# gogoex/BulletProofsPlus

Measured on AMD Instinct MI355X. Metric: aggregated range-proof verifies/sec (n=64,m=16), higher is better.
Workload: dtype u32 (30-bit limbs of a 381-bit prime field, v_mad_u64_u32)

## Files before the change

### bulletproofsplus_amd/csrc/ec.hpp

```cpp
#pragma once
#include "field.hpp"

namespace bpp {

struct Bls12381 {
    using Fp = BlsFp;
    using Fr = BlsFr;
    using K = Bls12381Consts;
    static constexpr int ID = 0;
};
struct Secp256k1 {
    using Fp = SecpFp;
    using Fr = SecpFr;
    using K = Secp256k1Consts;
    static constexpr int ID = 1;
};

template <class C>
constexpr int jac_words() {
    return 3 * C::Fp::N;
}

template <class C>
struct Aff {
    Fe<typename C::Fp> x, y;
    BPP_HD bool is_inf() const { return x.is_zero() && y.is_zero(); }
};

template <class C>
struct Jac {
    Fe<typename C::Fp> X, Y, Z;
    BPP_HD bool is_inf() const { return Z.is_zero(); }
};

template <class C>
BPP_HD Aff<C> aff_inf() {
    Aff<C> r;
    r.x = Fe<typename C::Fp>::zero();
    r.y = Fe<typename C::Fp>::zero();
    return r;
}
template <class C>
BPP_HD Jac<C> jac_inf() {
    Jac<C> r;
    r.X = Fe<typename C::Fp>::one();
    r.Y = Fe<typename C::Fp>::one();
    r.Z = Fe<typename C::Fp>::zero();
    return r;
}
template <class C>
BPP_HD Jac<C> jac_from_aff(const Aff<C>& p) {
    if (p.is_inf()) return jac_inf<C>();
    Jac<C> r;
// ... 237 lines not shown
    F Pp = fe_sub_nr<6>(U2, p.X);
    F R = fe_csub_nr<4>(S2, neg, p.Y);
    const F PP = fe_sqr_io(Pp);
    const F PPP = fe_mul(Pp, PP);
    const F Q = fe_mul(p.X, PP);
    const F u = fe_add_dbl_nr(PPP, Q);
    const F X3 = fe_sub_nr<4>(fe_sqr_io(R), u);
    const F T = fe_sub_nr<6>(Q, X3);
    const F nY = fe_sub_nr<2>(F::zero(), p.Y);
    const F ZZ3 = fe_mul(p.ZZ, PP);
#if defined(BPP_LAZY_CHECK) && !defined(__HIP_DEVICE_COMPILE__)
    BPP_LAZY_CHECK(fe_below_kp<2>(U2) && fe_below_kp<2>(S2) && fe_below_kp<8>(Pp) && fe_below_kp<6>(R) &&
                   fe_below_kp<2>(PP) && fe_below_kp<2>(PPP) && fe_below_kp<2>(Q) && fe_below_kp<4>(u) &&
                   fe_below_kp<6>(X3) && fe_below_kp<8>(T) && fe_below_kp<3>(nY) && fe_below_kp<2>(ZZ3));
#endif
    if (ZZ3.is_zero()) {
        if (fe_is_zero_mod<5>(R)) {
            Aff<C> qq;
            qq.x = qx;
            qq.y = neg ? fe_sub_nr<1>(F::zero(), qy) : qy;
            p = xyzz_dbl_aff(qq);
        } else {
            p = xyzz_inf<C>();
        }
        return;
    }
    p.Y = fe_mul_add(R, T, nY, PPP);
    p.X = X3;
    p.ZZZ = fe_mul(p.ZZZ, PPP);
    p.ZZ = ZZ3;
}

template <class C>
BPP_HD Jac<C> xyzz_to_jac(const Xyzz<C>& p) {
    if (p.is_inf()) return jac_inf<C>();
    Jac<C> r;
    r.X = fe_mul(p.X, p.ZZ);
    r.Y = fe_mul(p.Y, p.ZZZ);
    r.Z = p.ZZ;
    return r;
}

template <class C>
BPP_HD bool jac_is_identity_class(const Jac<C>& p) {
    return p.is_inf();
}

template <class C>
BPP_HD bool aff_in_prime_subgroup(const Aff<C>& p) {
    if constexpr (C::ID == 0) {
        using F = Fe<typename C::Fp>;
        if (p.is_inf()) return true;
        Jac<C> t = jac_inf<C>();
        for (int i = 63; i >= 0; i--) {
            t = jac_dbl(t);
            if ((C::K::ZABS >> i) & 1ull) t = jac_madd(t, p);
        }
        {
            const Jac<C> base = t;
            Jac<C> acc = jac_inf<C>();
            for (int i = 63; i >= 0; i--) {
                acc = jac_dbl(acc);
                if ((C::K::ZABS >> i) & 1ull) acc = jac_add(acc, base);
            }
            t = acc;
        }
// ... 244 lines not shown
    using F = Fe<typename C::Fp>;
    if (p.is_inf() || q.is_inf()) return p.is_inf() && q.is_inf();
    F Z1Z1 = fe_sqr(p.Z), Z2Z2 = fe_sqr(q.Z);
    if (fe_mul(p.X, Z2Z2) != fe_mul(q.X, Z1Z1)) return false;
    return fe_mul(fe_mul(p.Y, q.Z), Z2Z2) == fe_mul(fe_mul(q.Y, p.Z), Z1Z1);
}

template <class C>
BPP_HD Aff<C> aff_load(const uint32_t* w) {
    Aff<C> r;
    r.x = fe_load<typename C::Fp>(w);
    r.y = fe_load<typename C::Fp>(w + C::Fp::N);
    return r;
}
template <class C>
BPP_HD void aff_store(const Aff<C>& p, uint32_t* w) {
    fe_store(p.x, w);
    fe_store(p.y, w + C::Fp::N);
}
template <class C>
BPP_HD Jac<C> jac_load(const uint32_t* w) {
    Jac<C> r;
    r.X = fe_load<typename C::Fp>(w);
    r.Y = fe_load<typename C::Fp>(w + C::Fp::N);
    r.Z = fe_load<typename C::Fp>(w + 2 * C::Fp::N);
    return r;
}
template <class C>
BPP_HD void jac_store(const Jac<C>& p, uint32_t* w) {
    fe_store(p.X, w);
    fe_store(p.Y, w + C::Fp::N);
    fe_store(p.Z, w + 2 * C::Fp::N);
}

template <class C>
BPP_HD bool aff_from_wire(const uint32_t* w, Aff<C>& out) {
    constexpr int N = C::Fp::N;
    if (w[2 * N] | w[2 * N + 1]) {
        out = aff_inf<C>();
        return true;
    }
    if (!words_lt_mod<typename C::Fp>(w) || !words_lt_mod<typename C::Fp>(w + N)) return false;
    out.x = fe_from_canonical<typename C::Fp>(w);
    out.y = fe_from_canonical<typename C::Fp>(w + N);
    if (out.is_inf()) return false;
    return aff_on_curve(out);
}
template <class C>
BPP_HD void aff_to_wire(const Aff<C>& p, uint32_t* w) {
    constexpr int N = C::Fp::N;
    if (p.is_inf()) {
#pragma unroll
        for (int i = 0; i < 2 * N + 2; i++) w[i] = 0;
        w[2 * N] = 1;
        return;
    }
    fe_to_canonical(p.x, w);
    fe_to_canonical(p.y, w + N);
    w[2 * N] = 0;
    w[2 * N + 1] = 0;
}

template <class C>
BPP_HD Jac<C> aff_mul_words(const Aff<C>& p, const uint32_t* k, int nwords) {
    Jac<C> acc = jac_inf<C>();
    int top = nwords * 32 - 1;
// ... 10 lines not shown
```

### bulletproofsplus_amd/csrc/ed25519.hpp

```cpp
#pragma once
#include "ec.hpp"

namespace bpp {

struct Ed25519 {
    using Fp = EdFp;
    using Fr = EdFr;
    using K = Ed25519Consts;
    static constexpr int ID = 2;
};

template <>
constexpr int jac_words<Ed25519>() {
    return 4 * EdFp::N;
}

template <>
struct Aff<Ed25519> {
    Fe<EdFp> x, y;
    BPP_HD bool is_inf() const { return x.is_zero() && y == Fe<EdFp>::one(); }
};
template <>
struct Jac<Ed25519> {
    Fe<EdFp> X, Y, Z, T;
// ... 136 lines not shown
BPP_HD Xyzz<Ed25519> xyzz_dbl_aff(const Aff<Ed25519>& q) {
    Xyzz<Ed25519> r;
    r.e = aff_dbl(q);
    return r;
}
BPP_HD Xyzz<Ed25519> xyzz_madd(const Xyzz<Ed25519>& p, const Aff<Ed25519>& q) {
    Xyzz<Ed25519> r;
    r.e = jac_madd(p.e, q);
    return r;
}
BPP_HD void xyzz_madd_lazy(Xyzz<Ed25519>& p, const Aff<Ed25519>& q, bool neg) {
    using F = ed::F;
    Jac<Ed25519>& e = p.e;
    const F qm = fe_sub_nr<1>(q.y, q.x);
    const F qp = fe_add_nr(q.y, q.x);
    const F a1 = fe_sub_nr<2>(e.Y, e.X);
    const F b1 = fe_add_nr(e.Y, e.X);
    const F A = fe_mul(a1, ed::select(neg, qp, qm));
    const F B = fe_mul(b1, ed::select(neg, qm, qp));
    const F C = fe_mul(fe_mul(e.T, ed::konst(Ed25519Consts::D2)), fe_mul(q.x, q.y));
    const F D = fe_add_nr(e.Z, e.Z);
    F E = fe_sub_nr<2>(B, A);
    const F H = fe_add_nr(B, A);
    const F Fm = fe_sub_nr<2>(D, C);
    const F Gp = fe_add_nr(D, C);
    F Fq = ed::select(neg, Gp, Fm);
    F G = ed::select(neg, Fm, Gp);
    e.X = fe_mul_io(E, Fq);
    e.T = fe_mul(E, H);
    e.Y = fe_mul_io(G, H);
    e.Z = fe_mul(Fq, G);
}
BPP_HD Jac<Ed25519> xyzz_to_jac(const Xyzz<Ed25519>& p) { return p.e; }

template <>
BPP_HD Jac<Ed25519> jac_load<Ed25519>(const uint32_t* w) {
    constexpr int N = EdFp::N;
    Jac<Ed25519> r;
    r.X = fe_load<EdFp>(w);
    r.Y = fe_load<EdFp>(w + N);
    r.Z = fe_load<EdFp>(w + 2 * N);
    r.T = fe_load<EdFp>(w + 3 * N);
    return r;
}
BPP_HD void jac_store(const Jac<Ed25519>& p, uint32_t* w) {
    constexpr int N = EdFp::N;
    fe_store(p.X, w);
    fe_store(p.Y, w + N);
    fe_store(p.Z, w + 2 * N);
    fe_store(p.T, w + 3 * N);
}

template <>
BPP_HD bool aff_from_wire<Ed25519>(const uint32_t* w, Aff<Ed25519>& out) {
    constexpr int N = EdFp::N;
    if (w[2 * N] | w[2 * N + 1]) {
        out = aff_inf<Ed25519>();
        return true;
    }
    if (!words_lt_mod<EdFp>(w) || !words_lt_mod<EdFp>(w + N)) return false;
    out.x = fe_from_canonical<EdFp>(w);
    out.y = fe_from_canonical<EdFp>(w + N);
    return aff_on_curve(out);
}

}
```

### bulletproofsplus_amd/csrc/impl_msm.hpp

```cpp
#pragma once
#include "hash_to_group.hpp"
#include "host_util.hpp"
#include "pippenger.hpp"

namespace bpp {

template <class P>
__global__ void __launch_bounds__(64) k_dbg_field(int op, const uint32_t* a, const uint32_t* b, uint32_t* out, size_t n) {
    const size_t i = (size_t)blockIdx.x * blockDim.x + threadIdx.x;
    if (i >= n) return;
    uint32_t wa[P::N], wb[P::N], wr[P::N];
    for (int t = 0; t < P::N; t++) {
        wa[t] = a[i * P::N + t];
        wb[t] = b[i * P::N + t];
    }
    Fe<P> x = fe_from_canonical<P>(wa), y = fe_from_canonical<P>(wb), r;
    switch (op) {
        case 0: r = fe_mul(x, y); break;
        case 1: r = fe_add(x, y); break;
        case 2: r = fe_sub(x, y); break;
        case 3: r = fe_inv(x); break;
        case 4: r = fe_sqr(x); break;
        default: r = fe_neg(x); break;
    }
    fe_to_canonical(r, wr);
    for (int t = 0; t < P::N; t++) out[i * P::N + t] = wr[t];
}

template <class C>
__global__ void __launch_bounds__(64) k_dbg_point(int op, const uint32_t* a, const uint32_t* b, uint32_t* out, size_t n) {
    constexpr int WW = 2 * C::Fp::N + 2;
    const size_t i = (size_t)blockIdx.x * blockDim.x + threadIdx.x;
    if (i >= n) return;
    uint32_t wa[WW], wb[WW], wr[WW];
    for (int t = 0; t < WW; t++) {
        wa[t] = a[i * WW + t];
        wb[t] = b[i * WW + t];
    }
    Aff<C> p, q;
    aff_from_wire<C>(wa, p);
    aff_from_wire<C>(wb, q);
    Jac<C> r;
    switch (op) {
        case 0: r = jac_add(jac_from_aff(p), jac_from_aff(q)); break;
        case 1: r = jac_madd(jac_from_aff(p), q); break;
        case 2: r = jac_dbl(jac_from_aff(p)); break;
        case 3: r = jac_madd(jac_dbl(jac_from_aff(p)), q); break;
        case 4: r = jac_add(jac_dbl(jac_from_aff(p)), jac_dbl(jac_from_aff(q))); break;
        default: {
            Xyzz<C> acc = xyzz_inf<C>();
            acc = xyzz_madd(acc, p);
            acc = xyzz_madd(acc, q);
            acc = xyzz_madd(acc, p);
            r = xyzz_to_jac(acc);
            break;
        }
    }
    aff_to_wire(jac_to_aff(r), wr);
    for (int t = 0; t < WW; t++) out[i * WW + t] = wr[t];
}

template <class C>
struct MsmImpl {
    static constexpr int N = C::Fp::N;
    static constexpr int JW = jac_words<C>();
    static constexpr int WW = 2 * N + 2;
    static constexpr int PW = WW / 2;

    static int msm_batch_dev(const uint32_t* d_scalars, const uint32_t* d_points, const std::vector<uint64_t>& offsets,
                             uint64_t* out, hipStream_t st);

    static constexpr size_t PIPPENGER_MIN_N = 4096;
    static size_t msm_workspace_bytes(size_t n, int window_bits);
    static int msm_device(const uint32_t* d_scalars, const uint32_t* d_wire_points, size_t n, int window_bits,
                          uint32_t* d_out_wire, uint32_t* d_status, void* d_ws, size_t ws_bytes, hipStream_t st,
                          bpp_ctx* ctx = nullptr);

    static int msm_pippenger(const uint64_t* scalars, const uint64_t* points, size_t n, int window_bits, uint64_t* out);

    static int msm_batch(const uint64_t* scalars, const uint64_t* points, const uint32_t* lens, size_t count,
                         uint64_t* out);
// ... 317 lines not shown
```

### bulletproofsplus_amd/csrc/impl_prove_batch.hpp

```cpp
#pragma once
#include "impl_verify.hpp"
#include "prover_batch.hpp"

namespace bpp {

template <class C>
struct ProveBatchImpl {
    using V = VerifyImpl<C>;
    static constexpr int JW = V::JW, WW = V::WW;

    struct ProveLayout {
        size_t a, b, cG, cH, pwy, con, vps, part, part1, part2, vout, trst, ch, blind, vals, gams, total;
        size_t chunk;
        unsigned per;
    };
    static size_t prove_chunk(const VerifyShape& s, size_t count) {
        const uint32_t nvp = pb_num_vps(s.k, s.m);
        const size_t chunk_max = std::max<size_t>(1, std::min<size_t>(2048, ((size_t)12 << 30) / ((size_t)nvp * s.N * 32)));
        return std::min(chunk_max, std::max<size_t>(count, 1));
    }
    static ProveLayout prove_layout(const VerifyShape& s, size_t count, bool mixed = false) {
        ProveLayout w;
        const uint32_t nvp = pb_num_vps(s.k, s.m);
        w.chunk = prove_chunk(s, count);
        const size_t nv_total = w.chunk * nvp;
        w.per = blocks_per_proof(s, nv_total);
        const size_t vec = w.chunk * (size_t)s.mn * 32;
        WsCarver o;
        w.a = o.take(vec);
        w.b = o.take(vec);
        w.cG = o.take(vec);
        w.cH = o.take(vec);
        w.pwy = o.take(vec);
        w.con = o.take(w.chunk * (size_t)pb_consts_elems(s.k) * 32);
        w.vps = o.take(nv_total * (size_t)s.N * 32);
        w.part = o.take(nv_total * w.per * FIXED_BLOCK * JW * 4);
        w.part1 = o.take(nv_total * w.per * (FIXED_BLOCK / FOLD_GROUP) * JW * 4);
        w.part2 = o.take(nv_total * w.per * (FIXED_BLOCK / FOLD_GROUP / FOLD_GROUP2) * JW * 4);
        w.vout = o.take(w.chunk * (size_t)s.m * WW * 4);
        w.trst = o.take(w.chunk * 32);
        w.ch = o.take(w.chunk * (size_t)(3 + s.k) * 32);
        w.blind = o.take(w.chunk * (size_t)pb_blind_elems(s.k) * 32);
        w.vals = w.gams = 0;
        if (mixed) {
            w.vals = o.take(w.chunk * (size_t)s.m * 8);
            w.gams = o.take(w.chunk * (size_t)s.m * 32);
        }
        w.total = o.total;
        return w;
    }

    static ProverConsts literals() { return ProverConsts{0, 4, 5, 33, 44, 88, 123, 0}; }
    struct Chunk {
        const VerifyShape& s;
        const ProverConsts& pc;
        const ProveLayout& L;
        uint8_t* ws;
        size_t cnt;
        const uint32_t *blind, *px;
        uint32_t *o_pts, *o_V, *o_sc, *ch;
        hipStream_t st;
        const uint32_t* table;
        uint32_t* w(size_t off) const { return reinterpret_cast<uint32_t*>(ws + off); }
    };
    static void mulvec(const Chunk& c, VpSel sel);
    static const uint32_t* chunk_blinding(const uint32_t* slice, const uint8_t* blind_key, uint64_t index, uint32_t k, size_t cnt,
                                          const uint32_t* px, uint32_t* w_blind, hipStream_t st);
    static void argument(const Chunk& c, bool fs, VpSel literal_sel);

    static int prove_batch_device(bpp_verifier* v, const PassShape& ps, const uint64_t* d_values, const uint64_t* d_gammas,
// ... 59 lines not shown
                                           size_t count, int flags, const uint8_t* blind_key, uint64_t index_base,
                                           uint8_t* out_proofs, uint8_t* out_commitments);
    template <class F>
    static int prove_mixed_staged(const MixedPlan& p, const uint64_t* values, const uint64_t* gammas, size_t wsb, void* out0,
                                  size_t bytes0, void* out1, size_t bytes1, F&& run) {
        size_t nval = 0;
        for (uint32_t c = 0; c < MIXED_CLASSES; c++) nval += p.count[c] << c;
        DevBuf dv, dg, d0, d1, dws;
        HIPCHK(dv.alloc(nval * 8));
        HIPCHK(hipMemcpy(dv.p, values, nval * 8, hipMemcpyHostToDevice));
        int rc = upload_scalars<C>(gammas, nval, dg, nullptr);
        if (rc) return rc;
        HIPCHK(d0.alloc(bytes0));
        HIPCHK(d1.alloc(bytes1));
        HIPCHK(dws.alloc(wsb));
        rc = run(static_cast<const uint64_t*>(dv.p), static_cast<const uint64_t*>(dg.p), d0.p, d1.p, dws.p);
        if (rc) return rc;
        HIPCHK(hipDeviceSynchronize());
        HIPCHK(hipMemcpy(out0, d0.p, bytes0, hipMemcpyDeviceToHost));
        HIPCHK(hipMemcpy(out1, d1.p, bytes1, hipMemcpyDeviceToHost));
        return BPP_OK;
    }
};

#ifdef BPP_IMPL_DEFINITIONS
template <class C>
void ProveBatchImpl<C>::mulvec(const Chunk& c, VpSel sel) {
    const ProveLayout& L = c.L;
    const size_t nv = c.cnt * sel.cnt;
    const unsigned per = std::min(L.per, blocks_per_proof(c.s, nv));
    launch_fixed_msm<C, 2>((unsigned)(nv * per), c.st, c.s, c.w(L.vps), c.table, c.w(L.part), per, 0u, (const uint32_t*)nullptr,
                           (uint32_t*)nullptr, (size_t)0, 0u, sel);
    const size_t f1 = nv * per * (FIXED_BLOCK / FOLD_GROUP), f2 = f1 / FOLD_GROUP2;
    hipLaunchKernelGGL(k_partials_fold<C>, dim3(cdiv(f1, 64)), dim3(64), 0, c.st, c.w(L.part), FOLD_GROUP, c.w(L.part1), f1);
    hipLaunchKernelGGL(k_partials_fold<C>, dim3(cdiv(f2, 64)), dim3(64), 0, c.st, c.w(L.part1), FOLD_GROUP2, c.w(L.part2), f2);
    hipLaunchKernelGGL(k_pb_collect<C>, dim3(cdiv(nv, 64)), dim3(64), 0, c.st, c.s, sel, c.w(L.part2),
                       per * (FIXED_BLOCK / FOLD_GROUP / FOLD_GROUP2), c.o_pts, c.o_V, nv, c.px);
}

template <class C>
const uint32_t* ProveBatchImpl<C>::chunk_blinding(const uint32_t* slice, const uint8_t* blind_key, uint64_t index, uint32_t k,
                                                  size_t cnt, const uint32_t* px, uint32_t* w_blind, hipStream_t st) {
    if (slice || !blind_key) return slice;
    BlindKey bk;
    load_key_words(blind_key, bk.w);
    hipLaunchKernelGGL(k_pb_blind<C>, dim3(cdiv(cnt * pb_blind_elems(k), 64)), dim3(64), 0, st, bk, index, k, w_blind, cnt, px);
    return w_blind;
}

template <class C>
void ProveBatchImpl<C>::argument(const Chunk& c, bool fs, VpSel literal_sel) {
    const VerifyShape& s = c.s;
    const ProveLayout& L = c.L;
    const uint32_t k = s.k, nvp = pb_num_vps(k, s.m);
    const dim3 proofs((unsigned)c.cnt), lanes(cdiv(c.cnt, 64));
    auto round = [&](uint32_t t, uint32_t phase) {
        hipLaunchKernelGGL(k_pb_round<C>, proofs, dim3(256), 0, c.st, s, c.pc, c.blind, t, phase, c.w(L.a), c.w(L.b), c.w(L.cG),
                           c.w(L.cH), c.w(L.pwy), c.w(L.con), c.w(L.vps));
    };
    auto last = [&](uint32_t phase) {
        hipLaunchKernelGGL(k_pb_final<C>, proofs, dim3(256), 0, c.st, s, c.pc, c.blind, phase, c.w(L.a), c.w(L.b), c.w(L.cG),
                           c.w(L.cH), c.w(L.con), c.w(L.vps), c.o_sc, c.px);
    };
    if (!fs) {
        for (uint32_t t = 0; t < k; t++) round(t, PB_ALL);
        last(PB_ALL);
        mulvec(c, literal_sel);
        return;
// ... 213 lines not shown
```

### bulletproofsplus_amd/csrc/impl_verify.hpp

```cpp
#pragma once
#include <functional>
#include <memory>
#include <mutex>

#include "codec.hpp"
#include "combined.hpp"
#include "fixed_launch.hpp"
#include "host_util.hpp"
#include "mixed.hpp"
#include "pippenger.hpp"

enum { BPP_STAGE_FROM_WIRE = 0, BPP_STAGE_SCALARS, BPP_STAGE_FIXED_MSM, BPP_STAGE_VAR_MSM, BPP_STAGE_FINALIZE,
       BPP_NUM_STAGES };
constexpr int BPP_PROFILE_SLOTS = 64;

namespace bpp {
struct PassShape {
    VerifyShape s;
    const uint32_t* challenges;
    TranscriptState tr0;
};
}

struct bpp_verifier {
// ... 22 lines not shown
    }
};

namespace bpp {

inline unsigned blocks_per_proof(const VerifyShape& s, size_t count) {
    const unsigned maxb = cdiv(s.NF, FIXED_BLOCK);
    size_t tpp = ((size_t)1 << 18) / (count ? count : 1);
    tpp = std::max<size_t>(FIXED_BLOCK, std::min<size_t>(tpp, s.NF));
    const unsigned b_lat = cdiv(tpp, FIXED_BLOCK);
    const unsigned b_thr = std::min<unsigned>(cdiv((size_t)32768, count ? count : 1),
                                              std::max<unsigned>(1, s.NF / (FIXED_BLOCK * 4)));
#ifdef BPP_FORCE_PER
    if (count >= 1024) return std::max(1u, std::min<unsigned>(BPP_FORCE_PER, maxb));
#endif
    return std::max(1u, std::min(std::max(b_lat, b_thr), maxb));
}

#ifndef BPP_HORNER_TREE_MAX
#define BPP_HORNER_TREE_MAX 256
#endif
constexpr size_t HORNER_TREE_MAX = BPP_HORNER_TREE_MAX;
constexpr unsigned FOLD_GROUP = 8;
constexpr unsigned FOLD_GROUP2 = 4;

struct WsLayout {
    size_t pts, bad, scalars, prep, fthread, fpart, fpart2, fpart3, vpart, vdig, vwsum, vtbl, vscr, total;
};

template <class C>
struct VerifyImpl {
    static constexpr int N = C::Fp::N;
    static constexpr int JW = jac_words<C>();
    static constexpr int WW = 2 * N + 2;
    static constexpr int PW = WW / 2;

    static WsLayout ws_layout(const VerifyShape& s, size_t count) {
        WsLayout w;
        WsCarver o;
        w.pts = o.take(count * s.NV * 2 * N * 4);
        w.bad = o.take(count * 4);
        w.scalars = o.take(count * (size_t)s.N * 32);
        w.prep = o.take(count * vs_prep_bytes<C>(s));
        w.fthread = o.take(count * blocks_per_proof(s, count) * FIXED_BLOCK * JW * 4);
        w.fpart = o.take(count * blocks_per_proof(s, count) * (FIXED_BLOCK / FOLD_GROUP) * JW * 4);
        w.fpart2 = o.take(count * blocks_per_proof(s, count) * (FIXED_BLOCK / FOLD_GROUP / FOLD_GROUP2) * JW * 4);
        w.fpart3 = o.take(count * (FIXED_BLOCK / FOLD_GROUP / FOLD_GROUP2) * JW * 4);
        w.vpart = o.take(count * JW * 4);
        w.vdig = o.take(count * s.NV * VAR_DIGIT_STRIDE);
        w.vwsum = o.take(count * var_wsums_max<C>() * JW * 4);
        w.vtbl = o.take(count * s.NV * VAR_MULTIPLES * 2 * N * 4);
        w.vscr = o.take(count * s.NV * 2 * (VAR_MULTIPLES - 1) * N * 4);
        w.total = o.total;
        return w;
    }

    static int create(const bpp_ctx& ctx, const uint64_t* gh, const uint64_t* G, const uint64_t* H, size_t n, size_t m,
                      int window_bits, bpp_verifier** out);

    static PassShape own(const bpp_verifier* v) { return PassShape{v->s, v->challenges.u32(), v->tr0}; }
    static PassShape class_shape(const bpp_verifier* v, uint32_t c) {
        return c < v->views.size() ? v->views[c] : own(v);
    }

    static int run(bpp_verifier* v, const PassShape& ps, const uint64_t* d_points, const uint64_t* d_scalars, size_t count,
                   const uint64_t* d_challenges, uint32_t* d_ok, void* d_workspace, size_t workspace_bytes,
                   uint64_t* d_out_scalars, uint64_t* d_out_result, hipStream_t st);
    static int run(bpp_verifier* v, const uint64_t* d_points, const uint64_t* d_scalars, size_t count,
                   const uint64_t* d_challenges, uint32_t* d_ok, void* d_workspace, size_t workspace_bytes,
                   uint64_t* d_out_scalars, uint64_t* d_out_result, hipStream_t st) {
        return run(v, own(v), d_points, d_scalars, count, d_challenges, d_ok, d_workspace, workspace_bytes, d_out_scalars,
                   d_out_result, st);
    }

    static int range_scalars(const PassShape& ps, const uint64_t* d_scalars, const uint64_t* d_challenges, uint32_t* w_sc,
                             size_t count, uint32_t* w_prep, hipStream_t st) {
        const uint32_t* ch = d_challenges ? reinterpret_cast<const uint32_t*>(d_challenges) : ps.challenges;
        const uint32_t ch_stride = d_challenges ? (3 + ps.s.k) * 8 : 0;
        return launch_verify_scalars<C>(ps.s, reinterpret_cast<const uint32_t*>(d_scalars), ch, ch_stride, w_sc, count, w_prep, st);
// ... 559 lines not shown
    v->last_horner_form = lone ? 3u : tree;
    const size_t vlanes = count * (tree == 1 ? var_wsums<C>() * vgroups : var_windows<C>());
    HIPCHK(mark(ev, 2 * BPP_STAGE_VAR_MSM, st));
    hipLaunchKernelGGL(k_var_digits<C>, dim3(cdiv(npts, 256)), dim3(256), 0, st, s, w_sc, w_vd, npts, 0u);
    rc = join_tables(v, st, aux_lock);
    if (rc) return rc;
    hipLaunchKernelGGL(k_var_windows<C>, dim3(cdiv(vlanes, VAR_BLOCK)), dim3(VAR_BLOCK), 0, st, s, w_vd, w_vt, w_vw,
                       vlanes, tree == 1 ? 1u : 0u, vgroups);
    HIPCHK(mark(ev, 2 * BPP_STAGE_VAR_MSM + 1, st));
    return finish(v, s, ws, L, count, w_sc, w_vw, w_bad, d_ok, reinterpret_cast<uint32_t*>(d_out_result), tree, lone, st,
                  ev);
}

template <class C>
int VerifyImpl<C>::finish(bpp_verifier* v, const VerifyShape& s, uint8_t* ws, const WsLayout& L, size_t count,
                          const uint32_t* w_sc, const uint32_t* w_vw, const uint32_t* w_bad, uint32_t* d_ok,
                          uint32_t* d_out_result, uint32_t tree, bool lone, hipStream_t st, hipEvent_t* ev) {
    const unsigned bpp_ = blocks_per_proof(s, count);
    uint32_t* w_fp = reinterpret_cast<uint32_t*>(ws + L.fpart);
    uint32_t* w_vp = reinterpret_cast<uint32_t*>(ws + L.vpart);
    HIPCHK(mark(ev, 2 * BPP_STAGE_FIXED_MSM, st));
    const unsigned hb = tree == 1 ? (unsigned)count : cdiv(count, tree == 2 ? FIXED_BLOCK / 8 : FIXED_BLOCK);
    uint32_t* w_ft = reinterpret_cast<uint32_t*>(ws + L.fthread);
    launch_fixed_msm<C, 0>((unsigned)(hb + count * bpp_), st, s, w_sc, v->table.u32(), w_ft, bpp_, hb, w_vw, w_vp, count,
                           lone ? 3u : tree, VpSel{1u, 0u, 1u, 0u});
    HIPCHK(mark(ev, 2 * BPP_STAGE_FIXED_MSM + 1, st));
    HIPCHK(mark(ev, 2 * BPP_STAGE_FINALIZE, st));
    const unsigned folded = bpp_ * (FIXED_BLOCK / FOLD_GROUP);
    const unsigned folded2 = folded / FOLD_GROUP2;
    uint32_t* w_fp2 = reinterpret_cast<uint32_t*>(ws + L.fpart2);
    if (tree == 1) {
        if (!lone)
            hipLaunchKernelGGL(k_partials_fold<C>, dim3(cdiv(count * folded, 64)), dim3(64), 0, st, w_ft, FOLD_GROUP, w_fp,
                               count * folded);
        hipLaunchKernelGGL(k_finalize_tree<C>, dim3((unsigned)count), dim3(64), 0, st, lone ? w_ft : w_fp,
                           lone ? bpp_ : folded, w_vp, w_bad, d_ok, d_out_result, count);
        HIPCHK(mark(ev, 2 * BPP_STAGE_FINALIZE + 1, st));
        HIPCHK(hipGetLastError());
        return BPP_OK;
    }
    hipLaunchKernelGGL(k_partials_fold<C>, dim3(cdiv(count * folded, 64)), dim3(64), 0, st, w_ft, FOLD_GROUP, w_fp,
                       count * folded);
    hipLaunchKernelGGL(k_partials_fold<C>, dim3(cdiv(count * folded2, 64)), dim3(64), 0, st, w_fp, FOLD_GROUP2, w_fp2,
                       count * folded2);
    const uint32_t* w_last = w_fp2;
    unsigned last = folded2;
    if (bpp_ > 1) {
        uint32_t* w_fp3 = reinterpret_cast<uint32_t*>(ws + L.fpart3);
        last = folded2 / bpp_;
        hipLaunchKernelGGL(k_partials_fold<C>, dim3(cdiv(count * last, 64)), dim3(64), 0, st, w_fp2, bpp_, w_fp3,
                           count * last);
        w_last = w_fp3;
    }
    hipLaunchKernelGGL(k_finalize<C>, dim3(cdiv(count, 64)), dim3(64), 0, st, w_last, last, w_vp, 1u, w_bad, d_ok,
                       d_out_result, count);
    HIPCHK(mark(ev, 2 * BPP_STAGE_FINALIZE + 1, st));
    HIPCHK(hipGetLastError());
    return BPP_OK;
}

template <class C>
int VerifyImpl<C>::run_serialized(bpp_verifier* v, const uint8_t* d_proofs, const uint8_t* d_commitments, size_t count,
                                  bool transcript, uint32_t* d_ok, void* d_workspace, size_t workspace_bytes,
                                  hipStream_t st, uint32_t version, const GroupedArgs* grouped) {
    const VerifyShape& s = v->s;
    if (int rc = container_args_ok(v, version)) return rc;
    const SerLayout L = ser_layout(s, count, grouped ? grouped->group : 0u);
    if (workspace_bytes < L.total) return fail(BPP_E_ARG, "workspace too small");
    uint8_t* ws = static_cast<uint8_t*>(d_workspace);
    uint32_t* w_rec = reinterpret_cast<uint32_t*>(ws + L.records);
    uint32_t* w_sc = reinterpret_cast<uint32_t*>(ws + L.scalars);
    uint32_t* w_st = reinterpret_cast<uint32_t*>(ws + L.status);
    uint64_t* w_ch = reinterpret_cast<uint64_t*>(ws + L.challenges);
    HIPCHK(zero_words_async(w_st, count * 4, st));
    hipLaunchKernelGGL(k_container_decode<C>, dim3(cdiv(count * s.NV, 64)), dim3(64), 0, st, s, d_proofs, d_commitments,
                       w_rec, w_sc, w_st, count, version);
    if constexpr (C::ID == 0)
        hipLaunchKernelGGL(k_records_subgroup<C>, dim3(cdiv(count * s.NV, 64)), dim3(64), 0, st, w_rec, w_st, s.NV,
                           count * s.NV);
    HIPCHK(hipGetLastError());
    if (transcript) {
        int rc = derive_challenges(v, reinterpret_cast<const uint64_t*>(w_rec), count, w_ch, st);
        if (rc) return rc;
    }
// ... 413 lines not shown
```

### bulletproofsplus_amd/csrc/kernels.hpp

```cpp
#pragma once
#include <hip/hip_runtime.h>
#include "ec.hpp"
#include "fixed_glv.hpp"
#include "ed25519.hpp"
#include "ristretto.hpp"
#include "transcript.hpp"

namespace bpp {

constexpr unsigned MSM_BLOCK = 64;
constexpr unsigned VS_PB = 8;
constexpr unsigned VS_BLOCK = VS_PB * 64;
constexpr unsigned FIXED_BLOCK = 128;
constexpr unsigned VAR_BLOCK = 64;
template <class C>
constexpr bool var_glv() {
    return curve_has_glv<C>();
}
template <class C>
constexpr uint32_t var_windows() {
    return var_glv<C>() ? 33u : 65u;
}
template <class C>
constexpr uint32_t var_wsums() {
// ... 50 lines not shown
}

template <class C>
__device__ __forceinline__ Aff<C> aff_ldg(const uint32_t* __restrict__ p) {
    constexpr int N = C::Fp::N;
    constexpr int JW = jac_words<C>();
    uint32_t w[2 * N];
    ld_words<2 * N>(p, w);
    return aff_load<C>(w);
}
template <class C>
__device__ __forceinline__ void aff_stg(uint32_t* __restrict__ p, const Aff<C>& a) {
    constexpr int N = C::Fp::N;
    constexpr int JW = jac_words<C>();
    uint32_t w[2 * N];
    aff_store(a, w);
    st_words<2 * N>(p, w);
}
template <class C>
__device__ __forceinline__ Jac<C> jac_ldg(const uint32_t* __restrict__ p) {
    constexpr int N = C::Fp::N;
    constexpr int JW = jac_words<C>();
    uint32_t w[JW];
    ld_words<JW>(p, w);
    return jac_load<C>(w);
}
template <class C>
__device__ __forceinline__ void jac_stg(uint32_t* __restrict__ p, const Jac<C>& a) {
    constexpr int N = C::Fp::N;
    constexpr int JW = jac_words<C>();
    uint32_t w[JW];
    jac_store(a, w);
    st_words<JW>(p, w);
}

template <class C>
__device__ __forceinline__ Jac<C> block_reduce_jac(Jac<C> acc, uint32_t* lds) {
    constexpr int N = C::Fp::N;
    constexpr int JW = jac_words<C>();
    const int tid = threadIdx.x;
    for (int half = blockDim.x >> 1; half >= 1; half >>= 1) {
        if (tid >= half && tid < 2 * half) jac_store(acc, lds + (size_t)tid * JW);
        __syncthreads();
        if (tid < half) acc = jac_add(acc, jac_load<C>(lds + (size_t)(tid + half) * JW));
        __syncthreads();
    }
    return acc;
}

template <class T>
__device__ __forceinline__ T wave_shfl(const T& v, int src_lane) {
    static_assert(sizeof(T) % 4 == 0, "whole words");
    struct Words {
        uint32_t w[sizeof(T) / 4];
    };
    Words a = __builtin_bit_cast(Words, v);
#pragma unroll
    for (int i = 0; i < (int)(sizeof(T) / 4); i++) a.w[i] = (uint32_t)__shfl((int)a.w[i], src_lane, 64);
    return __builtin_bit_cast(T, a);
}

template <class C>
__device__ __forceinline__ Jac<C> wave_sum_jac(Jac<C> x, int span = 64) {
    const int lane = threadIdx.x & 63;
#pragma unroll 1
    for (int d = span >> 1; d >= 1; d >>= 1) {
// ... 722 lines not shown
__device__ __forceinline__ void glds16(const uint32_t* gsrc, uint32_t lds_byte_addr) {
    unsigned keep;
    lds_byte_addr = __builtin_amdgcn_readfirstlane(lds_byte_addr);
    asm volatile("s_mov_b32 %0, m0\n\ts_mov_b32 m0, %2\n\ts_nop 0\n\tglobal_load_lds_dwordx4 %1, off\n\ts_mov_b32 m0, %0"
                 : "=&s"(keep)
                 : "v"(gsrc), "s"(lds_byte_addr)
                 : "memory");
}

#ifndef BPP_FIXED_RING
#define BPP_FIXED_RING 2
#endif
constexpr int FIXED_RING = BPP_FIXED_RING;
template <class C>
constexpr unsigned fixed_lds_bytes() {
    return (FIXED_BLOCK / 64) * (FIXED_RING * (2 * C::Fp::N / 4) + 2) * 1024;
}

struct VpSel {
    uint32_t nvp, first, cnt, prover;
};

template <class C>
constexpr int fixed_waves() {
    return C::Fp::NL > 9 ? BPP_FIXED_WAVES : 3;
}
template <class C, int ROLE = 0>
__global__ void __launch_bounds__(FIXED_BLOCK, fixed_waves<C>()) k_fixed_msm(VerifyShape s, const uint32_t* __restrict__ scalars,
                            const uint32_t* __restrict__ table, uint32_t* __restrict__ partials, uint32_t per,
                            uint32_t horner_blocks, const uint32_t* __restrict__ wsum, uint32_t* __restrict__ var_out,
                            size_t horner_count, uint32_t horner_tree, VpSel sel) {
    constexpr int N = C::Fp::N;
    constexpr int JW = jac_words<C>();
    constexpr int CH = 2 * N / 4;
    constexpr int WAVE_WORDS = (FIXED_RING * CH + 2) * 256;
    constexpr bool GLV = fixed_glv<C>();
    constexpr int NWD = GLV ? GLV_HALF_WORDS : WIN_FULL_WORDS;
    extern __shared__ __align__(16) uint32_t lds[];
    if (blockIdx.x < horner_blocks) {
        if (horner_tree == 2) {
            const size_t b = (size_t)blockIdx.x * (blockDim.x / 8) + threadIdx.x / 8;
            var_horner_group<C>(wsum, var_out, b, b < horner_count, lds + (size_t)(threadIdx.x >> 6) * 64 * JW);
        } else if (horner_tree) {
            const size_t b = blockIdx.x;
            if constexpr (var_glv<C>()) {
                if (b < horner_count) var_horner_wave2<C>(wsum, var_out, b, lds, horner_tree == 3 ? VAR_GROUPS : 1u);
            } else {
                if (b < horner_count && threadIdx.x < 64) var_horner_wave_ed(wsum, var_out, b, horner_tree == 3 ? VAR_GROUPS : 1u);
            }
        } else {
            const size_t lane = (size_t)blockIdx.x * blockDim.x + threadIdx.x;
            if (lane < horner_count) var_horner_lane<C>(wsum, var_out, lane);
        }
        return;
    }
#ifdef BPP_XCD_REMAP
    uint32_t bid = blockIdx.x - horner_blocks;
    {
        const uint32_t nb = gridDim.x - horner_blocks;
        if (nb % 8 == 0 && horner_blocks % 8 == 0) bid = (bid % 8) * (nb / 8) + bid / 8;
    }
#else
    const uint32_t bid = blockIdx.x - horner_blocks;
#endif
    const size_t b = bid / per;
    const uint32_t part = bid % per;
// ... 148 lines not shown
        dma_scalar(0);
        asm volatile("s_waitcnt vmcnt(0)" ::: "memory");
        take_scalar();
        if (NQ > 1) dma_scalar(G > 1 ? 1u : 0u);
    }
    for (int d = 0; d < FIXED_RING; d++) issue();
    for (uint32_t ph = 0; ph < PH; ph++)
    for (uint32_t t = 0; t < (ph + 1 < PH ? T : TT); t++) {
        if constexpr (GLV) {
            if (ph == 1 && t == 0) xyzz_mul_x_beta(acc);
        }
        const uint32_t slot = (GLV ? ph * T + t : t) % FIXED_RING;
        asm volatile("s_waitcnt vmcnt(%0)" ::"n"((FIXED_RING - 1) * CH) : "memory");
        uint32_t raw[2 * N];
        const uint4* q = reinterpret_cast<const uint4*>(ring + slot * CH * 256);
#pragma unroll
        for (int k = 0; k < CH; k++) {
            const uint4 v = q[k * 64 + lane];
            raw[4 * k] = v.x;
            raw[4 * k + 1] = v.y;
            raw[4 * k + 2] = v.z;
            raw[4 * k + 3] = v.w;
        }
        const bool valid = (vbits >> slot) & 1u, neg = (nbits >> slot) & 1u;
        Aff<C> cur = aff_load<C>(raw);
        if constexpr (GLV) {
            if (ph == 1 && t >= T && ((bbits >> slot) & 1u)) aff_mul_x_beta(cur);
        }
        issue();
        if (valid) xyzz_madd_lazy(acc, cur, neg);
    }
    asm volatile("s_waitcnt vmcnt(0)" ::: "memory");
    if (ROLE != 1 && horner_tree != 3) {
        jac_stg<C>(partials + ((size_t)bid * blockDim.x + threadIdx.x) * JW, xyzz_to_jac(acc));
    } else {
        __syncthreads();
        Jac<C> sum = block_reduce_jac<C>(xyzz_to_jac(acc), lds);
        if (threadIdx.x == 0) jac_stg<C>(partials + (size_t)bid * JW, sum);
    }
}

template <class C>
__global__ void __launch_bounds__(64) k_partials_fold(const uint32_t* __restrict__ in, uint32_t group,
                                                      uint32_t* __restrict__ out, size_t n_out) {
    constexpr int JW = jac_words<C>();
    const size_t i = (size_t)blockIdx.x * blockDim.x + threadIdx.x;
    if (i >= n_out) return;
    const uint32_t* src = in + i * group * JW;
    Jac<C> acc = jac_ldg<C>(src);
    for (uint32_t t = 1; t < group; t++) acc = jac_add(acc, jac_ldg<C>(src + (size_t)t * JW));
    jac_stg<C>(out + i * JW, acc);
}


template <class C>
__global__ void __launch_bounds__(256) k_var_digits(VerifyShape s, const uint32_t* __restrict__ scalars,
                                                    uint8_t* __restrict__ digits, size_t items, uint32_t flat) {
    const size_t item = (size_t)blockIdx.x * blockDim.x + threadIdx.x;
    if (item >= items) return;
    const size_t b = item / s.NV;
    const uint32_t v = (uint32_t)(item % s.NV);
    uint32_t k[8];
    ld_words<8>(scalars + (flat ? item : b * s.N + var_term_index(s, v)) * 8, k);
    uint32_t out[VAR_DIGIT_STRIDE / 4];
#pragma unroll
    for (int t = 0; t < (int)(VAR_DIGIT_STRIDE / 4); t++) out[t] = 0;
    if constexpr (var_glv<C>()) {
        uint32_t rem[4], q[4];
        bool nh[2];
        glv_split_signed<C>(k, rem, q, nh[0], nh[1]);
#pragma unroll
        for (int h = 0; h < 2; h++) {
            uint32_t w[5];
            uint32_t carry = 0;
#pragma unroll
            for (int t = 0; t < 5; t++) {
                const uint64_t x = (uint64_t)(t < 4 ? (h ? q[t] : rem[t]) : 0u) + (t < 4 ? 0x88888888u : 0x8u) + carry;
                w[t] = (uint32_t)x;
                carry = (uint32_t)(x >> 32);
            }
#pragma unroll
            for (int j = 0; j < 33; j++) {
                uint32_t nib = (w[j >> 3] >> ((j & 7) * 4)) & 15u;
                if (nh[h]) nib = 16u - nib;
// ... 37 lines not shown
    uint32_t* T = tables + lane * M * 2 * N;
    uint32_t* S = scratch + lane * 2 * (M - 1) * N;
    const Aff<C> p = aff_ldg<C>(proof_pts + lane * 2 * N);
    aff_stg<C>(T, p);
    if (p.is_inf()) {
        for (int k = 1; k < M; k++) aff_stg<C>(T + (size_t)k * 2 * N, p);
        return;
    }
    affine_chain<C>(aff_dbl(p), T, M - 1, T + 2 * N, S);
}

template <class C>
__global__ void __launch_bounds__(VAR_BLOCK, BPP_VAR_WAVES) k_var_windows(VerifyShape s, const uint8_t* __restrict__ digits,
                                                                         const uint32_t* __restrict__ tables,
                                                                         uint32_t* __restrict__ wsum, size_t lanes,
                                                                         uint32_t split, uint32_t groups) {
    constexpr int N = C::Fp::N;
    constexpr int JW = jac_words<C>();
    const size_t lane = (size_t)blockIdx.x * blockDim.x + threadIdx.x;
    if (lane >= lanes) return;
    constexpr uint32_t NW = var_windows<C>();
    constexpr uint32_t H = var_glv<C>() ? 2u : 1u;
    const uint32_t HL = split ? 1u : H;
    const uint32_t per_proof = NW * (H / HL) * groups;
    const size_t b = lane / per_proof;
    const uint32_t g = (uint32_t)(lane % per_proof) / (NW * (H / HL));
    const uint32_t h0 = split ? (uint32_t)(lane / NW) % H : 0u;
    const uint32_t j = (uint32_t)(lane % NW);
    const uint32_t gs = (s.NV + groups - 1) / groups;
    const uint32_t v0 = g * gs, v1 = min(s.NV, v0 + gs);
    const uint8_t* dg = digits + b * s.NV * VAR_DIGIT_STRIDE + j;
    const uint32_t* T = tables + b * s.NV * VAR_MULTIPLES * 2 * N;
    Xyzz<C> acc = xyzz_inf<C>();
    Fe<typename C::Fp> beta;
    if constexpr (var_glv<C>()) {
#pragma unroll
        for (int i = 0; i < C::Fp::NL; i++) beta.l[i] = C::K::BETA[i];
    }
    const uint32_t items = (v1 > v0 ? v1 - v0 : 0u) * HL;
    auto digit_of = [&](uint32_t u) -> int32_t {
        return (int32_t)dg[(size_t)(v0 + u / HL) * VAR_DIGIT_STRIDE + (h0 + u % HL) * NW] - 8;
    };
    auto entry_of = [&](uint32_t u, int32_t d) -> const uint32_t* {
        return T + ((size_t)(v0 + u / HL) * VAR_MULTIPLES + (d < 0 ? -d : d) - 1) * 2 * N;
    };
    uint32_t raw[2 * N];
    int32_t d_next = items ? digit_of(0) : 0;
    if (d_next) ld_words<2 * N>(entry_of(0, d_next), raw);
    for (uint32_t u = 0; u < items; u++) {
        const int32_t d = d_next;
        Aff<C> cur;
        if (d) cur = aff_load<C>(raw);
        if (u + 1 < items) {
            d_next = digit_of(u + 1);
            if (d_next) ld_words<2 * N>(entry_of(u + 1, d_next), raw);
        }
        bool neg = d < 0;
        if constexpr (var_glv<C>()) {
            if (d && ((h0 + u % HL) & 1u)) {
                cur.x = fe_mul(cur.x, beta);
                fe_cond_sub_p(cur.x);
                if (glv_image_negates_y<C>()) neg = !neg;
            }
        }
        if (d) xyzz_madd_lazy(acc, cur, neg);
    }
    jac_stg<C>(wsum + lane * JW, xyzz_to_jac(acc));
}

template <class C>
__global__ void __launch_bounds__(64) k_finalize(const uint32_t* __restrict__ fixed_partials, uint32_t per,
                                                 const uint32_t* __restrict__ var_partials, uint32_t nv,
                                                 const uint32_t* __restrict__ bad, uint32_t* __restrict__ ok,
                                                 uint32_t* __restrict__ wire_result, size_t count) {
    constexpr int N = C::Fp::N;
    constexpr int JW = jac_words<C>();
    const size_t b = (size_t)blockIdx.x * blockDim.x + threadIdx.x;
    if (b >= count) return;
    Jac<C> acc = jac_inf<C>();
    for (uint32_t t = 0; t < per; t++) acc = jac_add(acc, jac_ldg<C>(fixed_partials + (b * per + t) * JW));
    for (uint32_t t = 0; t < nv; t++) acc = jac_add(acc, jac_ldg<C>(var_partials + (b * nv + t) * JW));
    ok[b] = (jac_is_identity_class(acc) && !bad[b]) ? 0u : 1u;
    if (wire_result) {
        uint32_t w[2 * N + 2];
        aff_to_wire(jac_to_aff(acc), w);
#pragma unroll
        for (int t = 0; t < 2 * N + 2; t++) wire_result[b * (2 * N + 2) + t] = w[t];
    }
}

template <class C>
__global__ void __launch_bounds__(64) k_finalize_tree(const uint32_t* __restrict__ fixed_partials, uint32_t per,
                                                      const uint32_t* __restrict__ var_partials,
                                                      const uint32_t* __restrict__ bad, uint32_t* __restrict__ ok,
                                                      uint32_t* __restrict__ wire_result, size_t count) {
    constexpr int N = C::Fp::N;
    constexpr int JW = jac_words<C>();
    __shared__ __align__(16) uint32_t lds[64 * JW];
// ... 18 lines not shown
```

Baseline: 202,500.

## Keep fixed-MSM partials in XYZZ form and batch GLV beta multiply

Fixed-base MSM threads now store their partial sums in XYZZ coordinates and the fold kernels add them with a new XYZZ+XYZZ addition. Conversion to Jacobian happens only at the last fold, which removes per-thread conversions and the costlier Jacobian additions. In the variable MSM the two GLV halves are iterated as separate contiguous runs. The endomorphism beta is then applied once to the accumulator at the end of the first half instead of to every looked-up point. Exchanges: partial buffers are a third larger (4 vs 3 field elements), and there is added lazy-reduction bookkeeping plus a debug test path.

```diff
diff --git a/bulletproofsplus_amd/csrc/ec.hpp b/bulletproofsplus_amd/csrc/ec.hpp
--- a/bulletproofsplus_amd/csrc/ec.hpp
+++ b/bulletproofsplus_amd/csrc/ec.hpp
@@ -19,6 +19,10 @@
 template <class C>
 constexpr int jac_words() {
     return 3 * C::Fp::N;
+}
+template <class C>
+constexpr int xyzz_words() {
+    return 4 * C::Fp::N;
 }
 
 template <class C>
@@ -322,6 +326,71 @@
 }
 
 template <class C>
+BPP_HD Xyzz<C> xyzz_dbl(const Xyzz<C>& p) {
+    using F = Fe<typename C::Fp>;
+    if (p.is_inf()) return xyzz_inf<C>();
+    F U = fe_dbl(p.Y);
+    F V = fe_sqr(U);
+    F W = fe_mul(U, V);
+    F S = fe_mul(p.X, V);
+    F xx = fe_sqr(p.X);
+    F M = fe_add(fe_dbl(xx), xx);
+    Xyzz<C> r;
+    r.X = fe_sub(fe_sqr(M), fe_dbl(S));
+    r.Y = fe_mul_add(M, fe_sub(S, r.X), fe_neg(W), p.Y);
+    r.ZZ = fe_mul(V, p.ZZ);
+    r.ZZZ = fe_mul(W, p.ZZZ);
+    return r;
+}
+template <class P>
+BPP_HD void fe_reduce_lazy(Fe<P>& a) {
+    fe_cond_sub<P>(a, P::MODK[4]);
+    fe_cond_sub<P>(a, P::MODK[2]);
+}
+template <class C>
+BPP_HD Xyzz<C> xyzz_add(const Xyzz<C>& p, const Xyzz<C>& q) {
+    using P = typename C::Fp;
+    using F = Fe<P>;
+    if (p.is_inf()) return q;
+    if (q.is_inf()) return p;
+    const F U1 = fe_mul(p.X, q.ZZ);
+    const F U2 = fe_mul(q.X, p.ZZ);
+    const F S1 = fe_mul(p.Y, q.ZZZ);
+    const F S2 = fe_mul(q.Y, p.ZZZ);
+    F Pp = fe_sub_nr<2>(U2, U1);
+    F R = fe_sub_nr<2>(S2, S1);
+    const F PP = fe_sqr_io(Pp);
+    const F PPP = fe_mul(Pp, PP);
+    const F Q = fe_mul(U1, PP);
+    const F u = fe_add_dbl_nr(PPP, Q);
+    const F X3 = fe_sub_nr<4>(fe_sqr_io(R), u);
+    const F T = fe_sub_nr<6>(Q, X3);
+    const F nS1 = fe_sub_nr<2>(F::zero(), S1);
+    const F ZZ3 = fe_mul(fe_mul(p.ZZ, q.ZZ), PP);
+#if defined(BPP_LAZY_CHECK) && !defined(__HIP_DEVICE_COMPILE__)
+    BPP_LAZY_CHECK(fe_below_kp<6>(p.X) && fe_below_kp<6>(q.X) && fe_below_kp<3>(p.Y) && fe_below_kp<3>(q.Y) &&
+                   fe_below_kp<2>(p.ZZ) && fe_below_kp<2>(q.ZZ) && fe_below_kp<2>(p.ZZZ) && fe_below_kp<2>(q.ZZZ) &&
+                   fe_below_kp<2>(U1) && fe_below_kp<2>(U2) && fe_below_kp<2>(S1) && fe_below_kp<2>(S2) &&
+                   fe_below_kp<4>(Pp) && fe_below_kp<4>(R) && fe_below_kp<2>(PP) && fe_below_kp<2>(PPP) &&
+                   fe_below_kp<2>(Q) && fe_below_kp<4>(u) && fe_below_kp<6>(X3) && fe_below_kp<8>(T) &&
+                   fe_below_kp<3>(nS1) && fe_below_kp<2>(ZZ3));
+#endif
+    if (ZZ3.is_zero()) {
+        if (!fe_is_zero_mod<3>(R)) return xyzz_inf<C>();
+        Xyzz<C> d = p;
+        fe_reduce_lazy(d.X);
+        fe_cond_sub<P>(d.Y, P::MODK[2]);
+        return xyzz_dbl(d);
+    }
+    Xyzz<C> r;
+    r.Y = fe_mul_add(R, T, nS1, PPP);
+    r.X = X3;
+    r.ZZZ = fe_mul(fe_mul(p.ZZZ, q.ZZZ), PPP);
+    r.ZZ = ZZ3;
+    return r;
+}
+
+template <class C>
 BPP_HD Jac<C> xyzz_to_jac(const Xyzz<C>& p) {
     if (p.is_inf()) return jac_inf<C>();
     Jac<C> r;
@@ -632,6 +701,26 @@
     fe_store(p.Y, w + C::Fp::N);
     fe_store(p.Z, w + 2 * C::Fp::N);
 }
+template <class C>
+BPP_HD Xyzz<C> xyzz_load(const uint32_t* w) {
+    Xyzz<C> r;
+    r.X = fe_load<typename C::Fp>(w);
+    r.Y = fe_load<typename C::Fp>(w + C::Fp::N);
+    r.ZZ = fe_load<typename C::Fp>(w + 2 * C::Fp::N);
+    r.ZZZ = fe_load<typename C::Fp>(w + 3 * C::Fp::N);
+    return r;
+}
+template <class C>
+BPP_HD void xyzz_store(const Xyzz<C>& p, uint32_t* w) {
+    using P = typename C::Fp;
+    Fe<P> x = p.X, y = p.Y;
+    fe_reduce_lazy(x);
+    fe_cond_sub<P>(y, P::MODK[2]);
+    fe_store(x, w);
+    fe_store(y, w + P::N);
+    fe_store(p.ZZ, w + 2 * P::N);
+    fe_store(p.ZZZ, w + 3 * P::N);
+}
 
 template <class C>
 BPP_HD bool aff_from_wire(const uint32_t* w, Aff<C>& out) {
diff --git a/bulletproofsplus_amd/csrc/ed25519.hpp b/bulletproofsplus_amd/csrc/ed25519.hpp
--- a/bulletproofsplus_amd/csrc/ed25519.hpp
+++ b/bulletproofsplus_amd/csrc/ed25519.hpp
@@ -192,6 +192,11 @@
     e.Z = fe_mul(Fq, G);
 }
 BPP_HD Jac<Ed25519> xyzz_to_jac(const Xyzz<Ed25519>& p) { return p.e; }
+BPP_HD Xyzz<Ed25519> xyzz_add(const Xyzz<Ed25519>& p, const Xyzz<Ed25519>& q) {
+    Xyzz<Ed25519> r;
+    r.e = jac_add(p.e, q.e);
+    return r;
+}
 
 template <>
 BPP_HD Jac<Ed25519> jac_load<Ed25519>(const uint32_t* w) {
@@ -210,6 +215,14 @@
     fe_store(p.Z, w + 2 * N);
     fe_store(p.T, w + 3 * N);
 }
+
+template <>
+BPP_HD Xyzz<Ed25519> xyzz_load<Ed25519>(const uint32_t* w) {
+    Xyzz<Ed25519> r;
+    r.e = jac_load<Ed25519>(w);
+    return r;
+}
+BPP_HD void xyzz_store(const Xyzz<Ed25519>& p, uint32_t* w) { jac_store(p.e, w); }
 
 template <>
 BPP_HD bool aff_from_wire<Ed25519>(const uint32_t* w, Aff<Ed25519>& out) {
diff --git a/bulletproofsplus_amd/csrc/impl_msm.hpp b/bulletproofsplus_amd/csrc/impl_msm.hpp
--- a/bulletproofsplus_amd/csrc/impl_msm.hpp
+++ b/bulletproofsplus_amd/csrc/impl_msm.hpp
@@ -25,6 +25,31 @@
     }
     fe_to_canonical(r, wr);
     for (int t = 0; t < P::N; t++) out[i * P::N + t] = wr[t];
+}
+
+template <class C>
+__device__ Xyzz<C> dbg_xyzz_scaled(const Aff<C>& a, uint32_t lam, bool lift) {
+    using P = typename C::Fp;
+    if (a.is_inf()) return xyzz_inf<C>();
+    const Fe<P> l = fe_from_u32<P>(lam), l2 = fe_sqr(l), l3 = fe_mul(l2, l);
+    Xyzz<C> r;
+    r.X = fe_mul(a.x, l2);
+    r.Y = fe_mul(a.y, l3);
+    r.ZZ = l2;
+    r.ZZZ = l3;
+    if (lift) {
+        Fe<P> m1, m5;
+#pragma unroll
+        for (int i = 0; i < P::NL; i++) {
+            m1.l[i] = P::MODK[1][i];
+            m5.l[i] = P::MODK[5][i];
+        }
+        fe_cond_sub_p(r.X);
+        fe_cond_sub_p(r.Y);
+        r.X = fe_add_nr(r.X, m5);
+        r.Y = fe_add_nr(r.Y, m1);
+    }
+    return r;
 }
 
 template <class C>
@@ -47,6 +72,19 @@
         case 2: r = jac_dbl(jac_from_aff(p)); break;
         case 3: r = jac_madd(jac_dbl(jac_from_aff(p)), q); break;
         case 4: r = jac_add(jac_dbl(jac_from_aff(p)), jac_dbl(jac_from_aff(q))); break;
+        case 6: {
+            if constexpr (C::ID == 2) {
+                r = jac_add(jac_from_aff(p), jac_from_aff(q));
+            } else {
+                const bool lift = ((i / 16) & 1u) != 0;
+                const Xyzz<C> xp = dbg_xyzz_scaled<C>(p, 1u + 7u * (uint32_t)(i % 4), lift);
+                const Xyzz<C> xq = dbg_xyzz_scaled<C>(q, 1u + 5u * (uint32_t)(i / 4 % 4), lift);
+                uint32_t w[xyzz_words<C>()];
+                xyzz_store(xyzz_add(xp, xq), w);
+                r = xyzz_to_jac(xyzz_load<C>(w));
+            }
+            break;
+        }
         default: {
             Xyzz<C> acc = xyzz_inf<C>();
             acc = xyzz_madd(acc, p);
diff --git a/bulletproofsplus_amd/csrc/impl_prove_batch.hpp b/bulletproofsplus_amd/csrc/impl_prove_batch.hpp
--- a/bulletproofsplus_amd/csrc/impl_prove_batch.hpp
+++ b/bulletproofsplus_amd/csrc/impl_prove_batch.hpp
@@ -34,8 +34,8 @@
         w.pwy = o.take(vec);
         w.con = o.take(w.chunk * (size_t)pb_consts_elems(s.k) * 32);
         w.vps = o.take(nv_total * (size_t)s.N * 32);
-        w.part = o.take(nv_total * w.per * FIXED_BLOCK * JW * 4);
-        w.part1 = o.take(nv_total * w.per * (FIXED_BLOCK / FOLD_GROUP) * JW * 4);
+        w.part = o.take(nv_total * w.per * FIXED_BLOCK * xyzz_words<C>() * 4);
+        w.part1 = o.take(nv_total * w.per * (FIXED_BLOCK / FOLD_GROUP) * xyzz_words<C>() * 4);
         w.part2 = o.take(nv_total * w.per * (FIXED_BLOCK / FOLD_GROUP / FOLD_GROUP2) * JW * 4);
         w.vout = o.take(w.chunk * (size_t)s.m * WW * 4);
         w.trst = o.take(w.chunk * 32);
@@ -161,8 +161,8 @@
     launch_fixed_msm<C, 2>((unsigned)(nv * per), c.st, c.s, c.w(L.vps), c.table, c.w(L.part), per, 0u, (const uint32_t*)nullptr,
                            (uint32_t*)nullptr, (size_t)0, 0u, sel);
     const size_t f1 = nv * per * (FIXED_BLOCK / FOLD_GROUP), f2 = f1 / FOLD_GROUP2;
-    hipLaunchKernelGGL(k_partials_fold<C>, dim3(cdiv(f1, 64)), dim3(64), 0, c.st, c.w(L.part), FOLD_GROUP, c.w(L.part1), f1);
-    hipLaunchKernelGGL(k_partials_fold<C>, dim3(cdiv(f2, 64)), dim3(64), 0, c.st, c.w(L.part1), FOLD_GROUP2, c.w(L.part2), f2);
+    hipLaunchKernelGGL(k_partials_fold<C>, dim3(cdiv(f1, 64)), dim3(64), 0, c.st, c.w(L.part), FOLD_GROUP, c.w(L.part1), f1, 0u);
+    hipLaunchKernelGGL(k_partials_fold<C>, dim3(cdiv(f2, 64)), dim3(64), 0, c.st, c.w(L.part1), FOLD_GROUP2, c.w(L.part2), f2, 1u);
     hipLaunchKernelGGL(k_pb_collect<C>, dim3(cdiv(nv, 64)), dim3(64), 0, c.st, c.s, sel, c.w(L.part2),
                        per * (FIXED_BLOCK / FOLD_GROUP / FOLD_GROUP2), c.o_pts, c.o_V, nv, c.px);
 }
diff --git a/bulletproofsplus_amd/csrc/impl_verify.hpp b/bulletproofsplus_amd/csrc/impl_verify.hpp
--- a/bulletproofsplus_amd/csrc/impl_verify.hpp
+++ b/bulletproofsplus_amd/csrc/impl_verify.hpp
@@ -78,6 +78,7 @@
 struct VerifyImpl {
     static constexpr int N = C::Fp::N;
     static constexpr int JW = jac_words<C>();
+    static constexpr int XW = xyzz_words<C>();
     static constexpr int WW = 2 * N + 2;
     static constexpr int PW = WW / 2;
 
@@ -88,9 +89,9 @@
         w.bad = o.take(count * 4);
         w.scalars = o.take(count * (size_t)s.N * 32);
         w.prep = o.take(count * vs_prep_bytes<C>(s));
-        w.fthread = o.take(count * blocks_per_proof(s, count) * FIXED_BLOCK * JW * 4);
-        w.fpart = o.take(count * blocks_per_proof(s, count) * (FIXED_BLOCK / FOLD_GROUP) * JW * 4);
-        w.fpart2 = o.take(count * blocks_per_proof(s, count) * (FIXED_BLOCK / FOLD_GROUP / FOLD_GROUP2) * JW * 4);
+        w.fthread = o.take(count * blocks_per_proof(s, count) * FIXED_BLOCK * XW * 4);
+        w.fpart = o.take(count * blocks_per_proof(s, count) * (FIXED_BLOCK / FOLD_GROUP) * XW * 4);
+        w.fpart2 = o.take(count * blocks_per_proof(s, count) * (FIXED_BLOCK / FOLD_GROUP / FOLD_GROUP2) * XW * 4);
         w.fpart3 = o.take(count * (FIXED_BLOCK / FOLD_GROUP / FOLD_GROUP2) * JW * 4);
         w.vpart = o.take(count * JW * 4);
         w.vdig = o.take(count * s.NV * VAR_DIGIT_STRIDE);
@@ -716,7 +717,7 @@
     if (tree == 1) {
         if (!lone)
             hipLaunchKernelGGL(k_partials_fold<C>, dim3(cdiv(count * folded, 64)), dim3(64), 0, st, w_ft, FOLD_GROUP, w_fp,
-                               count * folded);
+                               count * folded, 1u);
         hipLaunchKernelGGL(k_finalize_tree<C>, dim3((unsigned)count), dim3(64), 0, st, lone ? w_ft : w_fp,
                            lone ? bpp_ : folded, w_vp, w_bad, d_ok, d_out_result, count);
         HIPCHK(mark(ev, 2 * BPP_STAGE_FINALIZE + 1, st));
@@ -724,16 +725,16 @@
         return BPP_OK;
     }
     hipLaunchKernelGGL(k_partials_fold<C>, dim3(cdiv(count * folded, 64)), dim3(64), 0, st, w_ft, FOLD_GROUP, w_fp,
-                       count * folded);
+                       count * folded, 0u);
     hipLaunchKernelGGL(k_partials_fold<C>, dim3(cdiv(count * folded2, 64)), dim3(64), 0, st, w_fp, FOLD_GROUP2, w_fp2,
-                       count * folded2);
+                       count * folded2, bpp_ > 1 ? 0u : 1u);
     const uint32_t* w_last = w_fp2;
     unsigned last = folded2;
     if (bpp_ > 1) {
         uint32_t* w_fp3 = reinterpret_cast<uint32_t*>(ws + L.fpart3);
         last = folded2 / bpp_;
         hipLaunchKernelGGL(k_partials_fold<C>, dim3(cdiv(count * last, 64)), dim3(64), 0, st, w_fp2, bpp_, w_fp3,
-                           count * last);
+                           count * last, 1u);
         w_last = w_fp3;
     }
     hipLaunchKernelGGL(k_finalize<C>, dim3(cdiv(count, 64)), dim3(64), 0, st, w_last, last, w_vp, 1u, w_bad, d_ok,
diff --git a/bulletproofsplus_amd/csrc/kernels.hpp b/bulletproofsplus_amd/csrc/kernels.hpp
--- a/bulletproofsplus_amd/csrc/kernels.hpp
+++ b/bulletproofsplus_amd/csrc/kernels.hpp
@@ -106,6 +106,21 @@
     uint32_t w[JW];
     jac_store(a, w);
     st_words<JW>(p, w);
+}
+
+template <class C>
+__device__ __forceinline__ Xyzz<C> xyzz_ldg(const uint32_t* __restrict__ p) {
+    constexpr int XW = xyzz_words<C>();
+    uint32_t w[XW];
+    ld_words<XW>(p, w);
+    return xyzz_load<C>(w);
+}
+template <class C>
+__device__ __forceinline__ void xyzz_stg(uint32_t* __restrict__ p, const Xyzz<C>& a) {
+    constexpr int XW = xyzz_words<C>();
+    uint32_t w[XW];
+    xyzz_store(a, w);
+    st_words<XW>(p, w);
 }
 
 template <class C>
@@ -894,6 +909,7 @@
                             size_t horner_count, uint32_t horner_tree, VpSel sel) {
     constexpr int N = C::Fp::N;
     constexpr int JW = jac_words<C>();
+    constexpr int XW = xyzz_words<C>();
     constexpr int CH = 2 * N / 4;
     constexpr int WAVE_WORDS = (FIXED_RING * CH + 2) * 256;
     constexpr bool GLV = fixed_glv<C>();
@@ -1108,7 +1124,7 @@
     }
     asm volatile("s_waitcnt vmcnt(0)" ::: "memory");
     if (ROLE != 1 && horner_tree != 3) {
-        jac_stg<C>(partials + ((size_t)bid * blockDim.x + threadIdx.x) * JW, xyzz_to_jac(acc));
+        xyzz_stg<C>(partials + ((size_t)bid * blockDim.x + threadIdx.x) * XW, acc);
     } else {
         __syncthreads();
         Jac<C> sum = block_reduce_jac<C>(xyzz_to_jac(acc), lds);
@@ -1118,14 +1134,18 @@
 
 template <class C>
 __global__ void __launch_bounds__(64) k_partials_fold(const uint32_t* __restrict__ in, uint32_t group,
-                                                      uint32_t* __restrict__ out, size_t n_out) {
-    constexpr int JW = jac_words<C>();
+                                                      uint32_t* __restrict__ out, size_t n_out, uint32_t to_jac) {
+    constexpr int JW = jac_words<C>();
+    constexpr int XW = xyzz_words<C>();
     const size_t i = (size_t)blockIdx.x * blockDim.x + threadIdx.x;
     if (i >= n_out) return;
-    const uint32_t* src = in + i * group * JW;
-    Jac<C> acc = jac_ldg<C>(src);
-    for (uint32_t t = 1; t < group; t++) acc = jac_add(acc, jac_ldg<C>(src + (size_t)t * JW));
-    jac_stg<C>(out + i * JW, acc);
+    const uint32_t* src = in + i * group * XW;
+    Xyzz<C> acc = xyzz_ldg<C>(src);
+    for (uint32_t t = 1; t < group; t++) acc = xyzz_add(acc, xyzz_ldg<C>(src + (size_t)t * XW));
+    if (to_jac)
+        jac_stg<C>(out + i * JW, xyzz_to_jac(acc));
+    else
+        xyzz_stg<C>(out + i * XW, acc);
 }
 
 
@@ -1229,17 +1249,15 @@
     const uint8_t* dg = digits + b * s.NV * VAR_DIGIT_STRIDE + j;
     const uint32_t* T = tables + b * s.NV * VAR_MULTIPLES * 2 * N;
     Xyzz<C> acc = xyzz_inf<C>();
-    Fe<typename C::Fp> beta;
-    if constexpr (var_glv<C>()) {
-#pragma unroll
-        for (int i = 0; i < C::Fp::NL; i++) beta.l[i] = C::K::BETA[i];
-    }
-    const uint32_t items = (v1 > v0 ? v1 - v0 : 0u) * HL;
+    const uint32_t np = v1 > v0 ? v1 - v0 : 0u;
+    const uint32_t items = np * HL;
+    auto half_of = [&](uint32_t u) -> uint32_t { return HL == 2 ? (u < np ? 1u : 0u) : h0; };
+    auto point_of = [&](uint32_t u) -> uint32_t { return v0 + (u < np ? u : u - np); };
     auto digit_of = [&](uint32_t u) -> int32_t {
-        return (int32_t)dg[(size_t)(v0 + u / HL) * VAR_DIGIT_STRIDE + (h0 + u % HL) * NW] - 8;
+        return (int32_t)dg[(size_t)point_of(u) * VAR_DIGIT_STRIDE + half_of(u) * NW] - 8;
     };
     auto entry_of = [&](uint32_t u, int32_t d) -> const uint32_t* {
-        return T + ((size_t)(v0 + u / HL) * VAR_MULTIPLES + (d < 0 ? -d : d) - 1) * 2 * N;
+        return T + ((size_t)point_of(u) * VAR_MULTIPLES + (d < 0 ? -d : d) - 1) * 2 * N;
     };
     uint32_t raw[2 * N];
     int32_t d_next = items ? digit_of(0) : 0;
@@ -1254,13 +1272,12 @@
         }
         bool neg = d < 0;
         if constexpr (var_glv<C>()) {
-            if (d && ((h0 + u % HL) & 1u)) {
-                cur.x = fe_mul(cur.x, beta);
-                fe_cond_sub_p(cur.x);
-                if (glv_image_negates_y<C>()) neg = !neg;
-            }
+            if (glv_image_negates_y<C>() && half_of(u)) neg = !neg;
         }
         if (d) xyzz_madd_lazy(acc, cur, neg);
+        if constexpr (var_glv<C>()) {
+            if (half_of(u) && u + 1 == np) xyzz_mul_x_beta(acc);
+        }
     }
     jac_stg<C>(wsum + lane * JW, xyzz_to_jac(acc));
 }
```

Result: no change. 204,200, median of 6 (+0.8%).
